# DiWu9/Union-Thesis-SLAM

Hardware: AMD Instinct MI355X
Metric: depth frames/sec (640x480 into 512^3 @ 2 cm dense TSDF; hash alongside) (higher is better)
Workload: dtype f64

## Files before the change

### union-thesis-slam_amd/csrc/tsdf_common.hip

```cpp
#include <unistd.h>

#include <algorithm>
#include <atomic>
#include <chrono>
#include <cmath>
#include <condition_variable>
#include <cstring>
#include <mutex>
#include <thread>
#include <vector>

#include "tsdf_host.h"

namespace tsdf {

static thread_local std::string g_err;

int set_error(int code, const char* fmt, ...) {
    char buf[1024];
    va_list ap;
    va_start(ap, fmt);
    vsnprintf(buf, sizeof(buf), fmt, ap);
    va_end(ap);
    g_err = buf;
// ... 355 lines not shown
    CopyJob job_;
    std::atomic<unsigned long long> gen_{0};
    std::atomic<int> left_{0}, bad_{0}, sleepers_{0};
    int spin_us_ = 300;
};
}

extern "C" int tsdf_diag_depth_to_mm(const double* src, long long n, unsigned short* dst) {
    if (!src || !dst || n < 0) return set_error(TSDF_E_ARG, "bad arguments");
    return CopyPool::get().depth_mm(dst, src, (size_t)n) ? 1 : 0;
}

static void par_memcpy(void* dst, const void* src, size_t bytes) {
    if (bytes < (4u << 20)) {
        CopyPool::get().copy(dst, src, bytes);
        return;
    }
    const unsigned hw = std::thread::hardware_concurrency();
    const size_t nt = std::min<size_t>(8, hw ? hw : 1);
    std::vector<std::thread> th;
    const size_t chunk = (bytes + nt - 1) / nt;
    for (size_t i = 0; i < nt; ++i) {
        const size_t o = i * chunk;
        if (o >= bytes) break;
        th.emplace_back([=] { std::memcpy((char*)dst + o, (const char*)src + o, std::min(chunk, bytes - o)); });
    }
    for (auto& t : th) t.join();
}

int Base::prepare_batch(Batch* bt, const void* depth, int dk, const void* color, int ck, int H,
                        int W, const double K[9], const double* Tinv, const double* ow,
                        double ow_default, int flags, int first, int n, int slot) {
    TSDF_TRY(ensure_pyr(H, W));
    const size_t npx = (size_t)H * W;
    const size_t dbytes = npx * (dk == TSDF_DEPTH_U16_MM ? 2 : 8);
    const size_t cbytes = npx * (ck == TSDF_COLOR_RGB8 ? 3 : 4);
    const char* d = (const char*)depth + dbytes * (size_t)first;
    const char* c = (const char*)color + cbytes * (size_t)first;
    if (!(flags & TSDF_DEVICE_PTRS)) {
        if (prestaged >= 0) {
            slot = prestaged;
        } else {
            TSDF_TRY(stage_alloc(dbytes, cbytes));
            TSDF_HIP(hipEventSynchronize(ev_copied[slot]));
            par_memcpy(hst_depth[slot], d, dbytes * n);
            par_memcpy(hst_color[slot], c, cbytes * n);
        }
        const size_t c0 = prestaged >= 0 ? (size_t)std::min(pre_copied, n) : 0;
        TSDF_HIP(hipStreamWaitEvent(cstream, ev_free[slot], 0));
        if (c0 < (size_t)n) {
            TSDF_HIP(hipMemcpyAsync((char*)st_depth[slot] + dbytes * c0, (const char*)hst_depth[slot] + dbytes * c0,
                                    dbytes * (n - c0), hipMemcpyHostToDevice, cstream));
            TSDF_HIP(hipMemcpyAsync((char*)st_color[slot] + cbytes * c0, (const char*)hst_color[slot] + cbytes * c0,
                                    cbytes * (n - c0), hipMemcpyHostToDevice, cstream));
        }
        TSDF_HIP(hipEventRecord(ev_copied[slot], cstream));
        TSDF_HIP(hipStreamWaitEvent(stream, ev_copied[slot], 0));
        d = (const char*)st_depth[slot];
        c = (const char*)st_color[slot];
    }
    const bool mask = (flags & TSDF_DEPTH_INVALID_65535) && dk == TSDF_DEPTH_U16_MM;
    if (mask && (dmask_px < npx || !dmask_set[n_sets - 1])) {
        TSDF_TRY(sync_all());
        for (int k = 0; k < kSets; ++k) {
            if (dmask_set[k]) TSDF_HIP(hipFree(dmask_set[k]));
            dmask_set[k] = nullptr;
        }
        for (int k = 0; k < n_sets; ++k)
            TSDF_HIP(hipMalloc(&dmask_set[k], sizeof(unsigned short) * npx * batch));
        dmask_px = npx;
    }
    use_set(cur_set);
    bt->n = n;
    const bool tex = texel_now && dk == TSDF_DEPTH_U16_MM && ck == TSDF_COLOR_RGB8;
    bt->texel = tex ? 1 : 0;
    for (int i = 0; i < n; ++i) {
        Frame* fr = &bt->f[i];
        const double* T = Tinv + 16 * (size_t)(first + i);
        for (int r = 0; r < 12; ++r) fr->T[r] = T[r];
        fr->fx = (double)(float)K[0];
        fr->fy = (double)(float)K[4];
        fr->cx = (double)(float)K[2];
        fr->cy = (double)(float)K[5];
        const double margin = frame_margin(W, H, fr->cx, fr->cy);
        fr->half_m = 0.5 - margin;
        for (int j = 0; j < 4; ++j) {
            fr->Tf[j] = T[j] * fr->fx;
            fr->Tf[4 + j] = T[4 + j] * fr->fy;
        }
        {
            double wmax[3];
            for (int a = 0; a < 3; ++a) {
                const long long gmax = (a == 0 ? (long long)vol.off[0] + col_gx(vol, vol.nb[0] - 1) + kBrickEdge
                                               : (long long)vol.off[a] + vol.dims[a]);
                wmax[a] = fabs((double)vol.origin[a]) + vol.vs * (double)gmax + 1.0;
            }
            const double zmin = fold_bound(T, fr->fx, fr->fy, wmax, margin);
            long long bits;
            std::memcpy(&bits, &zmin, sizeof bits);
            const long long hi = (std::isfinite(zmin) && zmin < 1e300) ? (bits >> 32) + 1 : 0x7FEFFFFFll;
            fr->zmin_hi = (int)std::min<long long>(hi, 0x7FEFFFFFll);
        }
        fr->ow = ow ? ow[first + i] : ow_default;
        fr->ow32 = (float)fr->ow;
        fr->H = H;
        fr->W = W;
        fr->depth_src = d + dbytes * i;
        fr->depth_mask = mask ? dmask + npx * i : nullptr;
        fr->depth = mask ? (const void*)fr->depth_mask : fr->depth_src;
        fr->color = c + cbytes * i;
        const bool direct = ck == TSDF_COLOR_RGB8 && rgb_direct &&
                            (!(flags & TSDF_DEVICE_PTRS) || (call_color_end && (const char*)fr->color + cbytes < call_color_end));
        if (tex) fr->rgbx = rgbx + 2 * npx * i;
        else fr->rgbx = direct ? nullptr : rgbx + npx * i;
        fr->pyr = pyr + (size_t)lay.total * i;

        frustum_planes(fr, T, W, H);
    }
    for (int L = 0; L <= kPyrLevels; ++L) {
        bt->pg.off[L] = lay.off[L];
        bt->pg.w[L] = lay.w[L];
        bt->pg.h[L] = lay.h[L];
    }
    return TSDF_OK;
}

int Base::stage_alloc(size_t dbytes, size_t cbytes) {
    if (st_depth_bytes >= dbytes * batch && st_color_bytes >= cbytes * batch) return TSDF_OK;
    TSDF_TRY(sync_all());
    for (int k = 0; k < kSlots; ++k) {
        if (st_depth[k]) TSDF_HIP(hipFree(st_depth[k]));
        if (st_color[k]) TSDF_HIP(hipFree(st_color[k]));
        if (hst_depth[k]) TSDF_HIP(hipHostFree(hst_depth[k]));
        if (hst_color[k]) TSDF_HIP(hipHostFree(hst_color[k]));
        st_depth[k] = st_color[k] = hst_depth[k] = hst_color[k] = nullptr;
    }
    st_depth_bytes = st_color_bytes = 0;
    for (int k = 0; k < kSlots; ++k) {
        TSDF_HIP(hipMalloc(&st_depth[k], dbytes * batch));
        TSDF_HIP(hipMalloc(&st_color[k], cbytes * batch + 64));
        TSDF_HIP(hipHostMalloc(&hst_depth[k], dbytes * batch, hipHostMallocDefault));
        TSDF_HIP(hipHostMalloc(&hst_color[k], cbytes * batch, hipHostMallocDefault));
    }
    st_depth_bytes = dbytes * batch;
    st_color_bytes = cbytes * batch;
    return TSDF_OK;
}

bool Base::defer_same(int dk, int ck, int H, int W, const double* K) const {
    return dfr.dk_in == dk && dfr.ck == ck && dfr.H == H && dfr.W == W && std::memcmp(dfr.K, K, sizeof(dfr.K)) == 0;
}

int Base::defer_push(const void* depth, int dk, const void* color, int ck, int H, int W,
                     const double* K, const double* T, double ow) {
    const size_t cbytes = frame_bytes_color(ck, H, W), npx = (size_t)H * W;
    if (dfr.n == 0) {
        TSDF_TRY(stage_alloc(frame_bytes_depth(dk, H, W), cbytes));
        dfr.slot = defer_next;
        dfr.copied = 0;
        defer_next = (defer_next + 1) % kSlots;
        TSDF_HIP(hipEventSynchronize(ev_copied[dfr.slot]));
        dfr.dk_in = dk;
        dfr.dk = dk;
        dfr.ck = ck;
        dfr.H = H;
        dfr.W = W;
        std::memcpy(dfr.K, K, sizeof(dfr.K));
    }
    const int i = dfr.n;
    const bool try_mm = i == 0 ? mm_backoff == 0 : dfr.dk == TSDF_DEPTH_U16_MM;
    if (i == 0 && mm_backoff > 0) --mm_backoff;
    char* const cdst = (char*)hst_color[dfr.slot] + cbytes * i;
    if (dk == TSDF_DEPTH_F64_M && defer_mm && try_mm) {
        if (CopyPool::get().frame(true, (unsigned short*)hst_depth[dfr.slot] + npx * i, depth, npx, cdst, color,
                                  cbytes)) {
            dfr.dk = TSDF_DEPTH_U16_MM;
        } else {
            mm_backoff = kMmBackoff;
            if (i > 0) return kDeferFlush;
            dfr.dk = TSDF_DEPTH_F64_M;
            CopyPool::get().copy(hst_depth[dfr.slot], depth, frame_bytes_depth(dfr.dk, H, W));
        }
    } else {
        const size_t db = frame_bytes_depth(dfr.dk, H, W);
// ... 231 lines not shown
```

### union-thesis-slam_amd/csrc/tsdf_device.h

```cpp
#pragma once
#include <hip/hip_runtime.h>
#include <stdint.h>
#include <type_traits>

namespace tsdf {

constexpr int kBrickEdge = 8;
constexpr int kBrickVox = 512;
constexpr int kWG = 256;
constexpr int kPyrLevels = 6;
constexpr int kStatSpread = 64;
constexpr unsigned long long kEmpty = ~0ull;
constexpr unsigned long long kTomb = ~0ull - 1ull;

enum Stat { ST_VOXELS = 0, ST_VISITED, ST_TOUCHED, ST_ALLOC, ST_PROBE, ST_LOOKUPS, ST_OVERFLOW,
            ST_PROBE_MAX, ST_BAD_ENTRY, ST_UNIQUE, kNStat };

struct Vol {
    int dims[3];
    int off[3];
    int xstride;
    int xodd;
    int sb[3];
    int nb[3];
    int shard, n_shards;
    int canon;
    float origin[3];
    double vs, trunc;
    double rtrunc;
    const double* rcp;
};

__host__ __device__ inline int col_gx(const Vol& v, int c) {
    return (c >> 1) * 2 * v.xstride + (c & 1) * v.xodd;
}

struct Frame {
    double T[12];
    double fx, fy, cx, cy;
    double ow;
    double half_m;
    double Tf[8];
    int zmin_hi;
    float ow32;
    int H, W;
    const void* depth;
    const void* depth_src;
    unsigned short* depth_mask;
    const void* color;
    const unsigned* rgbx;
    const float* pyr;
    float planes[5][4];
    double eye[3];
};

struct PyrGeo {
    int off[kPyrLevels + 1];
    int w[kPyrLevels + 1];
    int h[kPyrLevels + 1];
};

#ifndef TSDF_MAX_BATCH
#define TSDF_MAX_BATCH 32
#endif
constexpr int kMaxBatch = TSDF_MAX_BATCH;
static_assert(kMaxBatch == 8 || kMaxBatch == 16 || kMaxBatch == 32, "frames per batch: 8, 16 or 32");
#ifndef TSDF_FULL_BATCH
#define TSDF_FULL_BATCH TSDF_MAX_BATCH
#endif
constexpr int kFullBatch = TSDF_FULL_BATCH < kMaxBatch ? TSDF_FULL_BATCH : kMaxBatch;
constexpr int kDoneWord = kMaxBatch + 8, kDoneWordC = kMaxBatch + 9, kCursorWord = kMaxBatch + 10;
constexpr int kCountWords = kMaxBatch + 16;
constexpr int kRcpTab = 4096;
constexpr int kRcpBig = 65536;

__device__ inline bool small_int(float w) {
    return w >= 0.0f && w < (float)(kRcpTab - kMaxBatch - 1) && w == truncf(w);
}
__device__ inline bool table_int(float w) {
    return w >= 0.0f && w < (float)(kRcpBig - kMaxBatch - 1) && w == truncf(w);
}
__device__ inline bool canon_color(float c) {
    return c >= 0.0f && c < 16777216.0f && c == truncf(c);
}
struct Batch {
    Frame f[kMaxBatch];
    PyrGeo pg;
    int n;
    int texel;
};

typedef unsigned long long ListEntry;

struct Pool {
    float* tsdf;
    float* weight;
    float* color;
};

struct PoolState {
    long long pool_top;
    long long free_count;
    long long cursor;
    long long n_overflow;
    long long tombs;
    long long n_inserted;
};

constexpr int kReports = 8;
struct PoolReport {
    long long pool_top, free_count, n_overflow;
    long long listed;
    long long tombs;
    long long seq;
};

struct Table {
    unsigned long long* keys;
    int* vals;
    unsigned long long* occ;
    int* free_list;
    ListEntry* overflow;
    PoolState* st;
    PoolReport* rb;
    long long capacity;
    long long shard_cap;
    long long max_blocks;
    const int* owned;
    int n_owned;
    int* ins_list;
    long long ins_cap;
    int overflow_cap;
    int int_bits;
};

template <bool POW2 = false>
__host__ __device__ inline long long ref_hash(long long x, long long y, long long z, long long n,
                                              int int_bits) {
    const unsigned long long P1 = 73856093ull, P2 = 19349669ull, P3 = 83492791ull;
    long long h;
    if (int_bits == 32) {
        const int a = (int)(unsigned)((unsigned long long)x * P1);
        const int b = (int)(unsigned)((unsigned long long)y * P2);
        const int c = (int)(unsigned)((unsigned long long)z * P3);
        h = (long long)(a ^ b ^ c);
    } else {
        h = (long long)(((unsigned long long)x * P1) ^ ((unsigned long long)y * P2) ^
                        ((unsigned long long)z * P3));
    }
    if (POW2 || (n & (n - 1)) == 0) return h & (n - 1);
    long long m = h % n;
    return m < 0 ? m + n : m;
}

template <bool POW2 = false>
__host__ __device__ inline int shard_of(long long home, int n_shards, long long cap) {
    if (POW2 || (cap & (cap - 1)) == 0) return (int)((home * n_shards) >> (63 - __builtin_clzll((unsigned long long)cap)));
    return (int)((home * n_shards) / cap);
}

__host__ __device__ inline unsigned long long pack_key(int bx, int by, int bz) {
    return (unsigned long long)bx | ((unsigned long long)by << 21) | ((unsigned long long)bz << 42);
}

__device__ inline int lane_id() { return threadIdx.x & 63; }

__device__ unsigned long long fcmp64_mask(double a, double b, int pred) __asm("llvm.amdgcn.fcmp.i64.f64");
__device__ unsigned long long fcmp32_mask(float a, float b, int pred) __asm("llvm.amdgcn.fcmp.i64.f32");
__device__ unsigned long long icmp32_mask(unsigned a, unsigned b, int pred) __asm("llvm.amdgcn.icmp.i64.i32");
constexpr int kCmpOGT = 2, kCmpOGE = 3, kCmpOLT = 4, kCmpUNE = 14, kCmpNE = 33, kCmpULT = 36, kCmpSGT = 38;
__device__ inline bool lane_in(unsigned long long m) { return __builtin_amdgcn_inverse_ballot_w64(m); }
__device__ inline void sel_in_place(float& x, float y, unsigned long long m) {
    asm("v_cndmask_b32 %0, %0, %1, %2" : "+v"(x) : "v"(y), "s"(m));
}

template <typename T>
__device__ inline T coh_load(T* p) {
    return __hip_atomic_load(p, __ATOMIC_RELAXED, __HIP_MEMORY_SCOPE_AGENT);
}
template <typename T>
__device__ inline void coh_store(T* p, T v) {
    __hip_atomic_store(p, v, __ATOMIC_RELAXED, __HIP_MEMORY_SCOPE_AGENT);
}

__device__ inline double vox_world(float origin, double vs, int g) {
    return (double)(float)((double)origin + vs * (double)g);
}

struct BrickBox {
    double p0[3];
    float ext[3];
    float ctr[3];
    float rad;
};

__device__ inline BrickBox brick_box(const Vol& v, const double* eye, int bx, int by, int bz, int nx = 1,
                                     int ny = 1, int nz = 1) {
    const int bb[3] = {bx, by, bz}, nn[3] = {nx, ny, nz};
    BrickBox r;
#pragma unroll
    for (int a = 0; a < 3; ++a) {
        const int lo = bb[a] * kBrickEdge;
        const int hi = min(lo + nn[a] * kBrickEdge - 1, v.dims[a] - 1);
        const int glo = (a == 0) ? col_gx(v, bb[0]) : lo;
        const int ghi = (a == 0) ? col_gx(v, hi >> 3) + (hi & 7) : hi;
        r.p0[a] = (double)v.origin[a] + v.vs * (double)(glo + v.off[a]);
        r.ext[a] = (float)(v.vs * (double)(ghi - glo));
        r.ctr[a] = (float)(r.p0[a] + 0.5 * v.vs * (double)(ghi - glo) - eye[a]);
    }
    r.rad = 0.5f * sqrtf(r.ext[0] * r.ext[0] + r.ext[1] * r.ext[1] + r.ext[2] * r.ext[2]) + 1e-4f;
    return r;
}

__device__ inline bool cull_brick(const Vol& v, const Frame& fr, const PyrGeo& pg, const BrickBox& bb) {
#pragma unroll
    for (int i = 0; i < 5; ++i) {
        const float* q = fr.planes[i];
        if (q[0] * bb.ctr[0] + q[1] * bb.ctr[1] + q[2] * bb.ctr[2] + q[3] < -bb.rad) return false;
    }
    const double* T = fr.T;
    float c0[3], d[3][3];
#pragma unroll
    for (int r = 0; r < 3; ++r) {
        c0[r] = (float)(T[4 * r + 0] * bb.p0[0] + T[4 * r + 1] * bb.p0[1] + T[4 * r + 2] * bb.p0[2] + T[4 * r + 3]);
#pragma unroll
        for (int a = 0; a < 3; ++a) d[r][a] = (float)T[4 * r + a] * bb.ext[a];
    }
    const float fx = (float)fr.fx, fy = (float)fr.fy, cx = (float)fr.cx, cy = (float)fr.cy;
    float zmin = 3e38f, zmax = -3e38f, umin = 3e38f, umax = -3e38f, vmin = 3e38f, vmax = -3e38f;
#pragma unroll
    for (int c = 0; c < 8; ++c) {
        float q[3];
#pragma unroll
        for (int r = 0; r < 3; ++r)
            q[r] = c0[r] + ((c & 1) ? d[r][0] : 0.0f) + ((c & 2) ? d[r][1] : 0.0f) + ((c & 4) ? d[r][2] : 0.0f);
        zmin = fminf(zmin, q[2]);
        zmax = fmaxf(zmax, q[2]);
        const float iz = __builtin_amdgcn_rcpf(fmaxf(q[2], 1e-6f));
        const float u = fx * q[0] * iz + cx, w = fy * q[1] * iz + cy;
        umin = fminf(umin, u); umax = fmaxf(umax, u);
        vmin = fminf(vmin, w); vmax = fmaxf(vmax, w);
    }
    if (zmax < -1e-4f) return false;
    int u0 = 0, u1 = fr.W - 1, v0 = 0, v1 = fr.H - 1;
    if (zmin > 0.2f) {
        const float fu0 = floorf(umin) - 1.0f, fu1 = ceilf(umax) + 1.0f;
        const float fv0 = floorf(vmin) - 1.0f, fv1 = ceilf(vmax) + 1.0f;
        if (fu1 < 0.0f || fv1 < 0.0f || fu0 > (float)(fr.W - 1) || fv0 > (float)(fr.H - 1)) return false;
        u0 = (int)fmaxf(fu0, 0.0f); u1 = (int)fminf(fu1, (float)(fr.W - 1));
        v0 = (int)fmaxf(fv0, 0.0f); v1 = (int)fminf(fv1, (float)(fr.H - 1));
    }
    int L = 1;
    while (L < kPyrLevels && (((u1 >> L) - (u0 >> L)) > 3 || ((v1 >> L) - (v0 >> L)) > 3)) ++L;
// ... 44 lines not shown
        unsigned long long tm = __ballot(kk == kTomb);
        if (emp) tm &= (emp & (~emp + 1)) - 1;
        if (tomb < 0 && tm) tomb = __shfl(s, __ffsll((long long)tm) - 1);
        if (emp) {
            if (!insert) return -1;
            const int le = __ffsll((long long)emp) - 1;
            const long long target = tomb >= 0 ? tomb : __shfl(s, le);
            const unsigned long long expect = tomb >= 0 ? kTomb : kEmpty;
            int ok = 0;
            if (lane == 0) {
                if (blk < 0) blk = pool_alloc(t);
                if (blk >= 0) {
                    const unsigned long long old = atomicCAS(&t.keys[target], expect, key);
                    if (old == expect) {
                        coh_store(&t.vals[target], blk);
                        ok = 1;
                    } else if (old == key) {
                        ok = 2;
                    }
                }
            }
            blk = __shfl(blk, 0);
            ok = __shfl(ok, 0);
            if (blk == -2) return -1;
            if (ok == 1) {
                is_new = true;
                slot_out = target;
                probe = scanned + ((target - pos + t.capacity) % t.capacity);
                return blk;
            }
            if (ok == 2) {
                slot_out = target;
                probe = scanned + ((target - pos + t.capacity) % t.capacity);
                return coh_load(&t.vals[target]);
            }
            scanned += (target - pos + t.capacity) % t.capacity + 1;
            pos = target + 1;
            if (pos >= t.capacity) pos -= t.capacity;
            tomb = -1;
            continue;
        }
        pos += 64;
        if (pos >= t.capacity) pos -= t.capacity;
        scanned += 64;
    }
    return -1;
}


__device__ unsigned short buf_ld_u16(__amdgpu_buffer_rsrc_t r, int vindex, int voffset, int soffset,
                                     int aux) __asm("llvm.amdgcn.struct.ptr.buffer.load.i16");
__device__ unsigned buf_ld_u32(__amdgpu_buffer_rsrc_t r, int vindex, int voffset, int soffset,
                               int aux) __asm("llvm.amdgcn.struct.ptr.buffer.load.i32");
__device__ double buf_ld_f64(__amdgpu_buffer_rsrc_t r, int vindex, int voffset, int soffset,
                             int aux) __asm("llvm.amdgcn.struct.ptr.buffer.load.f64");
constexpr int kBufDword3 = 0x00020000;
typedef unsigned u32x2 __attribute__((ext_vector_type(2)));
__device__ u32x2 buf_ld_v2u32(__amdgpu_buffer_rsrc_t r, int vindex, int voffset, int soffset,
                              int aux) __asm("llvm.amdgcn.struct.ptr.buffer.load.v2i32");
struct FrameBufs {
    __amdgpu_buffer_rsrc_t depth, color;
};
template <int DK, int CK>
__device__ inline FrameBufs frame_bufs(const Frame& fr) {
    const int n = fr.W * fr.H;
    FrameBufs b;
    if (DK == 2) {
        static_assert(DK != 2 || CK == 0, "texels: RGB8 colour");
        b.depth = b.color = __builtin_amdgcn_make_buffer_rsrc((void*)fr.rgbx, 8, n, kBufDword3);
        return b;
    }
    b.depth = __builtin_amdgcn_make_buffer_rsrc((void*)fr.depth, DK == 0 ? 2 : 8, n, kBufDword3);
    if (CK == 0 && !fr.rgbx) b.color = __builtin_amdgcn_make_buffer_rsrc((void*)fr.color, 3, n, kBufDword3);
    else b.color = __builtin_amdgcn_make_buffer_rsrc((void*)(CK == 0 ? (const void*)fr.rgbx : fr.color), 4, n, kBufDword3);
    return b;
}
template <int DK>
__device__ inline unsigned depth_raw(const FrameBufs& fb, unsigned p) {
    return DK == 0 ? (unsigned)buf_ld_u16(fb.depth, (int)p, 0, 0, 0) : 0u;
}
template <int DK>
__device__ inline double depth_m(const FrameBufs& fb, unsigned p, unsigned raw) {
    if (DK != 1) {
        const double m = (double)raw;
        return fma(m, 0.001, m * -2.0858186326137145e-20);
    }
    return buf_ld_f64(fb.depth, (int)p, 0, 0, 0);
}

__device__ inline double div_rn(double a, double b, double y) {
    const double q0 = a * y;
    const double r = fma(-q0, b, a);
    return fma(r, y, q0);
}

__device__ inline float div_rn32(float a, float b, float y) {
    const float q0 = a * y;
    const float r = fmaf(-q0, b, a);
    return fmaf(r, y, q0);
}

typedef float f2 __attribute__((ext_vector_type(2)));
__device__ inline f2 pk_fma(f2 a, f2 b, f2 c) { return __builtin_elementwise_fma(a, b, c); }
__device__ inline f2 rint2(f2 a) { return f2{rintf(a.x), rintf(a.y)}; }
__device__ inline f2 div_rn32x2(f2 a, f2 b, f2 y) {
    const f2 q0 = a * y;
    const f2 r = pk_fma(-q0, b, a);
    return pk_fma(r, y, q0);
}

inline double frame_margin(int W, int H, double cx, double cy) {
    const double span = (double)(W > H ? W : H) + fmax(fabs(cx), fabs(cy));
    return fmax(1e-4, 1e-7 * span);
}

inline double fold_bound(const double* T, double fx, double fy, const double wmax[3], double margin) {
    double e = 0.0;
    for (int r = 0; r < 2; ++r) {
        const double* t = T + 4 * r;
        const double s = fabs(t[0]) * wmax[0] + fabs(t[1]) * wmax[1] + fabs(t[2]) * wmax[2] + fabs(t[3]);
        e = fmax(e, 8.0 * 0x1p-53 * (r == 0 ? fx : fy) * s);
    }
    return 4.0 * e / margin;
}

__device__ inline int cvt_i32_sat(double x) {
    int r;
    asm("v_cvt_i32_f64 %0, %1" : "=v"(r) : "v"(x));
    return r;
}

__device__ inline double readlane_f64(double x, int l) {
    const unsigned long long u = __double_as_longlong(x);
    const unsigned lo = __builtin_amdgcn_readlane((unsigned)u, l);
    const unsigned hi = __builtin_amdgcn_readlane((unsigned)(u >> 32), l);
    return __longlong_as_double(((long long)hi << 32) | lo);
}


#ifdef TSDF_DIAG
__device__ unsigned long long g_ddiag[8];
#define TSDF_DDIAG(i) (lane_id() == 0 ? (void)atomicAdd(&g_ddiag[i], 1ull) : (void)0)
#else
#define TSDF_DDIAG(i) ((void)0)
#endif

template <int DK, int CK, int NZ>
__device__ __forceinline__ void project_part(double trunc, const Frame& fr, double px, double py,
                                             const double* pzs, double pz_l, int zoff, unsigned long long colm,
                                             int nz, unsigned (&cpx)[NZ], double (&diff)[NZ],
                                             unsigned long long (&okm)[NZ]) {
    constexpr int kPz = NZ < 8 ? NZ : 1;
    const double a2 = fma(fr.T[9], py, fr.T[8] * px);
    const double b0 = fma(fr.Tf[1], py, fma(fr.Tf[0], px, fr.Tf[3]));
    const double b1 = fma(fr.Tf[5], py, fma(fr.Tf[4], px, fr.Tf[7]));
    double zc[NZ];
    int iu[NZ], iv[NZ];
    unsigned long long in[NZ], slow[NZ], any_slow = 0;
#pragma unroll
    for (int k = 0; k < NZ; ++k) {
        const double pz = NZ < 8 ? pzs[k % kPz] : readlane_f64(pz_l, k + zoff);
        zc[k] = fr.T[11] + fma(fr.T[10], pz, a2);
    }
    double rzs[NZ];
#pragma unroll
    for (int k = 0; k < NZ; ++k) rzs[k] = __builtin_amdgcn_rcp(zc[k]);
#pragma unroll
    for (int k = 0; k < NZ; ++k) {
        const double pz = NZ < 8 ? pzs[k % kPz] : readlane_f64(pz_l, k + zoff);
        const double z = zc[k], rz = rzs[k];
        const double sx = fma(fma(fr.Tf[2], pz, b0), rz, fr.cx), sy = fma(fma(fr.Tf[6], pz, b1), rz, fr.cy);
        const double ux = rint(sx), uy = rint(sy);
        const unsigned long long fine = fcmp64_mask(fabs(sx - ux), fr.half_m, kCmpOLT) &
                                        fcmp64_mask(fabs(sy - uy), fr.half_m, kCmpOLT) &
                                        icmp32_mask((unsigned)(__double_as_longlong(z) >> 32), (unsigned)fr.zmin_hi, kCmpSGT);
        const unsigned long long col = k < nz ? colm : 0ull;
        in[k] = col & fine;
        iu[k] = cvt_i32_sat(ux);
        iv[k] = cvt_i32_sat(uy);
        slow[k] = col & ~fine;
        any_slow |= slow[k];
    }
    TSDF_DDIAG(0);
    if (any_slow) {
        TSDF_DDIAG(3);
        const double a0 = fma(fr.T[1], py, fr.T[0] * px);
        const double a1 = fma(fr.T[5], py, fr.T[4] * px);
#pragma unroll
        for (int k = 0; k < NZ; ++k) {
            slow[k] &= fcmp64_mask(zc[k], 0.0, kCmpOGT);
            in[k] |= slow[k];
            if (!slow[k] || !lane_in(slow[k])) continue;
            TSDF_DDIAG(2);
            const double pz = NZ < 8 ? pzs[k % kPz] : readlane_f64(pz_l, k + zoff);
            const double x = fr.T[3] + fma(fr.T[2], pz, a0);
            const double y = fr.T[7] + fma(fr.T[6], pz, a1);
            iu[k] = cvt_i32_sat(rint((x * fr.fx) / zc[k] + fr.cx));
            iv[k] = cvt_i32_sat(rint((y * fr.fy) / zc[k] + fr.cy));
        }
    }
    unsigned long long cand[NZ];
    unsigned pix[NZ];
    const int W = fr.W, H = fr.H;
#pragma unroll
    for (int k = 0; k < NZ; ++k) {
        cand[k] = in[k] & icmp32_mask((unsigned)iu[k], (unsigned)W, kCmpULT) &
                  icmp32_mask((unsigned)iv[k], (unsigned)H, kCmpULT);
        pix[k] = lane_in(cand[k]) ? __umul24((unsigned)iv[k], (unsigned)W) + (unsigned)iu[k] : 0u;
    }
    const FrameBufs fb = frame_bufs<DK, CK>(fr);
    unsigned draw[NZ];
#pragma unroll
    for (int k = 0; k < NZ; ++k) {
        if (DK == 2) {
            const u32x2 t = buf_ld_v2u32(fb.depth, (int)pix[k], 0, 0, 0);
            draw[k] = t.x;
            cpx[k] = t.y;
        } else {
            draw[k] = depth_raw<DK>(fb, pix[k]);
            cpx[k] = buf_ld_u32(fb.color, (int)pix[k], 0, 0, 0);
        }
    }
    __builtin_amdgcn_sched_barrier(0);
    double dep[NZ];
#pragma unroll
    for (int k = 0; k < NZ; ++k) dep[k] = depth_m<DK>(fb, pix[k], draw[k]);
#pragma unroll
    for (int k = 0; k < NZ; ++k) {
        diff[k] = dep[k] - zc[k];
        const unsigned long long dpos = DK != 1 ? icmp32_mask(draw[k], 0u, kCmpNE) : fcmp64_mask(dep[k], 0.0, kCmpOGT);
        okm[k] = cand[k] & dpos & fcmp64_mask(diff[k], -trunc, kCmpOGE);
    }
}

__device__ inline double dist_of(double trunc, double rtrunc, double diff) {
    return fmin(div_rn(diff, trunc, rtrunc), 1.0);
}

constexpr int kResFree = -1, kResFail = -3;

template <bool HASH, int DK, int CK, bool OW1, int NZ, bool CU = false>
__device__ inline void integrate_brick(const Vol& v, const Batch& bt, const Pool& pool,
                                       const Table& tab, ListEntry entry, int zoff,
                                       unsigned long long* s_stat, const double* s_rcp,
                                       unsigned& nupd, unsigned& nuniq, int* res = nullptr) {
    static_assert(!CU || (CK == 0 && OW1), "u32 colour registers: RGB8 frames, obs_weight 1");
    static_assert(NZ == 8 || NZ == 4, "z-parts of 8 or 4 steps");
    constexpr bool kHalfHash = HASH && NZ == 4;
    const int lane = lane_id();
    const int b = __builtin_amdgcn_readfirstlane((int)(entry & 0xFFFFFFFFull));
    const unsigned fmask = __builtin_amdgcn_readfirstlane((unsigned)(entry >> 32));
    const double trunc = v.trunc, rtrunc = v.rtrunc;
    const double* const rcp_hbm = v.rcp;
    const bool canon = CU || v.canon != 0;
    const int nb12 = v.nb[1] * v.nb[2];
    if (b >= v.nb[0] * nb12) {
        if (lane == 0) atomicAdd(&s_stat[ST_BAD_ENTRY], 1ull);
        return;
    }
    const int bx = b / nb12;
    const int rem = b - bx * nb12;
    const int by = rem / v.nb[2];
    const int bz = rem - by * v.nb[2];
    const int lx = bx * kBrickEdge + (lane >> 3);
    const int ly = by * kBrickEdge + (lane & 7);
    const unsigned long long colm = __ballot(lx < v.dims[0] && ly < v.dims[1]);
    const int nz = min(kBrickEdge, v.dims[2] - bz * kBrickEdge) - zoff;
    const double px = vox_world(v.origin[0], v.vs, v.off[0] + col_gx(v, bx) + (lane >> 3));
    const double py = vox_world(v.origin[1], v.vs, v.off[1] + ly);
    const double pz_l = vox_world(v.origin[2], v.vs, v.off[2] + bz * kBrickEdge + (lane & 7));
    constexpr int kPz = NZ < 8 ? NZ : 1;
    double pzs[kPz];
#pragma unroll
    for (int k = 0; k < kPz; ++k) {
        pzs[k] = readlane_f64(pz_l, k + zoff);
        if (NZ < 8) asm("" : "+v"(pzs[k]));
    }

    typename std::conditional<HASH, int, long long>::type blk = HASH ? -1 : b;
    bool is_new = false;
    bool upd = false;
    if constexpr (kHalfHash) {
        const int cur = __builtin_amdgcn_readfirstlane(res[b]);
        if (cur == kResFail) {
            if (zoff == 0 && lane == 0) {
                const unsigned long long o = atomicAdd((unsigned long long*)&tab.st->n_overflow, 1ull);
                if ((long long)o < tab.overflow_cap) tab.overflow[o] = entry;
                atomicAdd(&s_stat[ST_OVERFLOW], 1ull);
            }
            return;
        }
        if (cur < 0 || cur >= tab.max_blocks) {
            if (lane == 0) atomicAdd(&s_stat[ST_BAD_ENTRY], 1ull);
            return;
        }
        blk = cur;
    }
    float ws[NZ], ts[NZ], cs[NZ];
#pragma unroll
    for (int k = 0; k < NZ; ++k) {
        ws[k] = 0.0f;
        ts[k] = 1.0f;
        cs[k] = 0.0f;
    }
    constexpr int kH = NZ / 4;
    unsigned long long loaded[kH];
#pragma unroll
    for (int h = 0; h < kH; ++h) loaded[h] = 0;
    unsigned long long touched[NZ] = {};
    bool w_small = true;
    bool w_table = true;
    bool c_canon = true;
    bool fast_t = OW1 && s_rcp, table_t = false, fast_c = CK == 0 && fast_t;
// ... 673 lines not shown
#endif
#ifndef TSDF_HASH_WAVES
#define TSDF_HASH_WAVES 4
#endif
template <bool HASH, int DK, int CK, bool OW1, int NZ = 8>
__global__ __launch_bounds__(kWG) __attribute__((amdgpu_waves_per_eu(TSDF_HASH_WAVES))) void k_integrate(Vol v, Batch bt, Pool pool, Table tab,
                                                  unsigned long long* stats, const ListEntry* list,
                                                  unsigned int* count, int n_list) {
    (void)v;
    const Vol& vk = *(const Vol*)opaque((VolP)__builtin_amdgcn_kernarg_segment_ptr());
    __shared__ unsigned long long s_stat[kNStat];
    __shared__ double s_rcp[OW1 ? kRcpTab : 1];
    __shared__ unsigned s_next;
    const int tid = threadIdx.x;
    if (tid < kNStat) s_stat[tid] = 0;
    if (tid == 0) s_next = 0;
    if (OW1)
        for (int i = tid; i < kRcpTab / 2; i += kWG) ((double2*)s_rcp)[i] = ((const double2*)vk.rcp)[i];
    __syncthreads();
    integrate_list<HASH, DK, CK, OW1, NZ>(vk, bt, pool, tab, list, count, n_list,
                                          blockIdx.x * (kWG / 64) + (tid >> 6), gridDim.x * (kWG / 64),
                                          s_stat, OW1 ? s_rcp : nullptr, &s_next, blockIdx.x, gridDim.x);
    __syncthreads();
    flush_stats(s_stat, stats);
}

template <int REDUCE>
__device__ inline void pyr_level(const PyrGeo& pg, float* pyr, int L, const float (*src)[33],
                                 float (*dst)[33], int n, int tx = blockIdx.x, int ty = blockIdx.y) {
    const int t = threadIdx.x;
    if (t < n * n) {
        const int rr = t / n, cc = t - rr * n;
        const float m = fmaxf(fmaxf(src[2 * rr][2 * cc], src[2 * rr][2 * cc + 1]),
                              fmaxf(src[2 * rr + 1][2 * cc], src[2 * rr + 1][2 * cc + 1]));
        dst[rr][cc] = m;
        const int X = tx * n + cc, Y = ty * n + rr;
        if (X < pg.w[L] && Y < pg.h[L]) pyr[pg.off[L] + Y * pg.w[L] + X] = m;
    }
}

template <int DK = 0>
__device__ inline void prep_vec_tile(const Batch& bt, unsigned int* count, int tx, int ty, int tf,
                                     float (*sa)[33], float (*sb)[33]) {
    const Frame& fr = bt.f[tf];
    float* pyr = (float*)fr.pyr;
    const int t = threadIdx.x, r = t >> 4, c = t & 15;
    if (count && t < kCountWords && tx == 0 && ty == 0 && tf == 0) coh_store(count + t, 0u);
    const bool act = t < 512;
    const int x0 = tx * 64 + c * 4, y0 = ty * 64 + r * 2;
    float ma = 0.0f, mb = 0.0f;
    if (act && x0 < fr.W) {
#pragma unroll
        for (int dy = 0; dy < 2; ++dy) {
            const int y = y0 + dy;
            if (y >= fr.H) continue;
            const size_t p = (size_t)y * fr.W + x0;
            uint2 dd = make_uint2(0u, 0u);
            if (DK == 1) {
                const double2 d0 = *(const double2*)((const double*)fr.depth_src + p);
                const double2 d1 = *(const double2*)((const double*)fr.depth_src + p + 2);
                ma = fmaxf(ma, fmaxf((float)d0.x, (float)d0.y));
                mb = fmaxf(mb, fmaxf((float)d1.x, (float)d1.y));
            } else {
                dd = *(const uint2*)((const unsigned short*)fr.depth_src + p);
                if (fr.depth_mask) {
                    unsigned lo0 = dd.x & 0xFFFFu, hi0 = dd.x >> 16, lo1 = dd.y & 0xFFFFu, hi1 = dd.y >> 16;
                    lo0 = lo0 == 65535u ? 0u : lo0;
                    hi0 = hi0 == 65535u ? 0u : hi0;
                    lo1 = lo1 == 65535u ? 0u : lo1;
                    hi1 = hi1 == 65535u ? 0u : hi1;
                    dd = make_uint2(lo0 | (hi0 << 16), lo1 | (hi1 << 16));
                    *(uint2*)(fr.depth_mask + p) = dd;
                }
                ma = fmaxf(ma, fmaxf((float)(dd.x & 0xFFFFu) * 1e-3f, (float)(dd.x >> 16) * 1e-3f));
                mb = fmaxf(mb, fmaxf((float)(dd.y & 0xFFFFu) * 1e-3f, (float)(dd.y >> 16) * 1e-3f));
            }
            if (fr.rgbx) {
                const unsigned* q = (const unsigned*)((const unsigned char*)fr.color + 3 * p);
                const unsigned a = q[0], b = q[1], cc = q[2];
                const uint4 c4 = make_uint4(a & 0xFFFFFFu, (a >> 24) | ((b & 0xFFFFu) << 8),
                                            (b >> 16) | ((cc & 0xFFu) << 16), cc >> 8);
                if (DK == 2) {
                    uint4* t = (uint4*)((uint2*)fr.rgbx + p);
                    t[0] = make_uint4(dd.x & 0xFFFFu, c4.x, dd.x >> 16, c4.y);
                    t[1] = make_uint4(dd.y & 0xFFFFu, c4.z, dd.y >> 16, c4.w);
                } else {
                    *(uint4*)((unsigned*)fr.rgbx + p) = c4;
                }
            }
        }
    }
    const PyrGeo& pg = bt.pg;
    const auto put = [&](int L, int X, int Y, float m) {
        if (X < pg.w[L] && Y < pg.h[L]) pyr[pg.off[L] + Y * pg.w[L] + X] = m;
    };
    if (act) {
        const int X = x0 >> 1, Y = y0 >> 1;
        put(1, X, Y, ma);
        put(1, X + 1, Y, mb);
    }
    float m2 = fmaxf(ma, mb);
    m2 = fmaxf(m2, __shfl_down(m2, 16));
    if (act && (r & 1) == 0) put(2, tx * 16 + c, ty * 16 + (r >> 1), m2);
    float m3 = fmaxf(m2, __shfl_down(m2, 1));
    m3 = fmaxf(m3, __shfl_down(m3, 32));
    if (act && (r & 3) == 0 && (c & 1) == 0) {
        put(3, tx * 8 + (c >> 1), ty * 8 + (r >> 2), m3);
        sa[r >> 2][c >> 1] = m3;
    }
    __syncthreads();
    if (t < 64) {
        const int lx = t & 7, ly = t >> 3;
        float m = sa[ly][lx];
        m = fmaxf(m, __shfl_down(m, 1));
        m = fmaxf(m, __shfl_down(m, 8));
        if ((lx & 1) == 0 && (ly & 1) == 0) put(4, tx * 4 + (lx >> 1), ty * 4 + (ly >> 1), m);
        m = fmaxf(m, __shfl_down(m, 2));
        m = fmaxf(m, __shfl_down(m, 16));
        if ((lx & 3) == 0 && (ly & 3) == 0) put(5, tx * 2 + (lx >> 2), ty * 2 + (ly >> 2), m);
        m = fmaxf(m, __shfl_down(m, 4));
        m = fmaxf(m, __shfl_down(m, 32));
        if (t == 0) put(6, tx, ty, m);
    }
    (void)sb;
}

template <int DK = 0>
__global__ __launch_bounds__(512) void k_prep_vec(Batch bt, unsigned int* count) {
    __shared__ float sa[32][33];
    __shared__ float sb[32][33];
    prep_vec_tile<DK>(bt, count, blockIdx.x, blockIdx.y, blockIdx.z, sa, sb);
}

template <int DK, int CK>
__global__ __launch_bounds__(1024) void k_prep(Batch bt, unsigned int* count) {
    __shared__ float sa[32][33];
    __shared__ float sb[32][33];
    const Frame& fr = bt.f[blockIdx.z];
    float* pyr = (float*)fr.pyr;
    unsigned* rgbx = (unsigned*)fr.rgbx;
    const int t = threadIdx.x, r = t >> 5, c = t & 31;
    if (count && t < kCountWords && blockIdx.x == 0 && blockIdx.y == 0 && blockIdx.z == 0) coh_store(count + t, 0u);
    const int x0 = blockIdx.x * 64 + c * 2, y0 = blockIdx.y * 64 + r * 2;
    float m1 = 0.0f;
#pragma unroll
    for (int dy = 0; dy < 2; ++dy)
#pragma unroll
        for (int dx = 0; dx < 2; ++dx) {
            const int x = x0 + dx, y = y0 + dy;
            if (x < fr.W && y < fr.H) {
                const int p = y * fr.W + x;
                float d;
                if (DK == 0) {
                    unsigned v = ((const unsigned short*)fr.depth_src)[p];
                    if (fr.depth_mask) {
                        v = (v == 65535u) ? 0u : v;
                        fr.depth_mask[p] = (unsigned short)v;
                    }
                    d = (float)v * 1e-3f;
                } else {
                    d = (float)((const double*)fr.depth_src)[p];
                }
                if (CK == 0 && rgbx) {
                    const unsigned char* q = (const unsigned char*)fr.color + 3 * (size_t)p;
                    const unsigned c = (unsigned)q[0] | ((unsigned)q[1] << 8) | ((unsigned)q[2] << 16);
                    rgbx[p] = c;
                }
                m1 = fmaxf(m1, (float)d);
// ... 220 lines not shown
```

### union-thesis-slam_amd/csrc/tsdf_host.h

```cpp
#pragma once
#include <hip/hip_runtime.h>

#include <cstdarg>
#include <cstdlib>
#include <cstdio>
#include <string>
#include <utility>
#include <vector>

#include "tsdf_device.h"
#include "tsdf_hip.h"

#ifndef TSDF_CULL_WAVES_DEFAULT
#define TSDF_CULL_WAVES_DEFAULT 2
#endif

namespace tsdf {

int set_error(int code, const char* fmt, ...);

#define TSDF_HIP(expr)                                                                        \
    do {                                                                                      \
        hipError_t e_ = (expr);                                                               \
        if (e_ != hipSuccess)                                                                 \
            return ::tsdf::set_error(e_ == hipErrorOutOfMemory ? TSDF_E_OOM : TSDF_E_HIP,     \
                                     "%s failed: %s (%s:%d)", #expr, hipGetErrorString(e_),   \
                                     __FILE__, __LINE__);                                     \
    } while (0)

#define TSDF_TRY(expr)            \
    do {                          \
        int r_ = (expr);          \
        if (r_ != TSDF_OK) return r_; \
    } while (0)

inline size_t frame_bytes_depth(int dk, int H, int W) { return (size_t)H * W * (dk == TSDF_DEPTH_U16_MM ? 2 : 8); }
inline size_t frame_bytes_color(int ck, int H, int W) { return (size_t)H * W * (ck == TSDF_COLOR_RGB8 ? 3 : 4); }

struct PyrLayout {
    int off[kPyrLevels + 1];
    int w[kPyrLevels + 1];
    int h[kPyrLevels + 1];
    int total;
};
PyrLayout pyr_layout(int H, int W);

struct Profiler {
    bool on = false;
    std::vector<std::pair<hipEvent_t, hipEvent_t>> pending;
    std::vector<hipEvent_t> spare;
    double ms = 0.0;
    long long launches = 0;
    int begin(hipStream_t s, hipEvent_t* e0);
    int end(hipStream_t s, hipEvent_t e0);
    int collect();
    void release();
};

constexpr int kSets = 3;
constexpr int kSlots = 4;

struct IcpCtx;
void icp_ctx_free(IcpCtx* c);

struct Base {
    int device = 0;
    hipStream_t stream = nullptr;
    Vol vol{};
    Pool pool{};
    long long n_bricks = 0;
    int batch = kMaxBatch;
    int set_batch(int want);
    int defer_frames = 8;
    int dma_grain = 2;
    bool rgb_direct = true;
    int texel_mode = -1;
    bool texel_now = false;
    static constexpr long long kTexelMinBricksDense = 3ll << 14, kTexelMinBricksHash = 3ll << 15;
    bool texel_for(int dk, long long owned_bricks, long long min_bricks) const {
        if (dk != TSDF_DEPTH_U16_MM) return false;
        return texel_mode >= 0 ? texel_mode != 0 : owned_bricks >= min_bricks;
    }
    bool defer_mm = true;
    int mm_backoff = 0;
    static constexpr int kMmBackoff = 4;
    const char* call_color_end = nullptr;
    float* pyr = nullptr;
    unsigned* rgbx = nullptr;
    int pyr_H = 0, pyr_W = 0;
    ListEntry* list = nullptr;
    unsigned int* count = nullptr;
    float* pyr_set[kSets] = {};
    unsigned* rgbx_set[kSets] = {};
    ListEntry* list_set[kSets] = {};
    unsigned int* count_set[kSets] = {};
    unsigned short* dmask_set[kSets] = {};
    int n_sets = 1;
    int n_cu = 256;
    PyrLayout lay{};
    unsigned long long* stats = nullptr;
    double* rcp = nullptr;
    long long frames = 0;
    Profiler prof;
    hipStream_t cstream = nullptr;
    hipEvent_t ev_copied[kSlots] = {};
    hipEvent_t ev_free[kSlots] = {};
    void* st_depth[kSlots] = {};
    void* st_color[kSlots] = {};
    size_t st_depth_bytes = 0, st_color_bytes = 0;
    unsigned short* dmask = nullptr;
    size_t dmask_px = 0;
    void* hst_depth[kSlots] = {};
    void* hst_color[kSlots] = {};

    struct Deferred {
        int n = 0, H = 0, W = 0, dk = 0, ck = 0, slot = -1;
        int dk_in = 0;
        int copied = 0;
        double K[9];
        double T[16 * kMaxBatch];
        double ow[kMaxBatch];
    } dfr;
    int defer_next = 0;
    int prestaged = -1;
    int pre_copied = 0;
    bool defer_same(int dk, int ck, int H, int W, const double* K) const;
    int defer_push(const void* depth, int dk, const void* color, int ck, int H, int W,
                   const double* K, const double* T, double ow);
    static constexpr int kDeferFlush = 1;
    int stage_alloc(size_t dbytes, size_t cbytes);
    bool stage_fits(int dk, int ck, int H, int W) const {
        return st_depth_bytes >= frame_bytes_depth(dk, H, W) * batch &&
               st_color_bytes >= frame_bytes_color(ck, H, W) * batch;
    }

    int init(int dev, const int64_t dims[3], const int64_t off[3], const float origin[3],
             double vs, double trunc);
    int use_sets(int n);
    int cur_set = 0;
    void use_set(int s) {
        cur_set = s;
        pyr = pyr_set[s];
        rgbx = rgbx_set[s];
        list = list_set[s];
        count = count_set[s];
        dmask = dmask_set[s];
    }
    int sync_all();
    int ensure_pyr(int H, int W);
    int prepare_batch(Batch* bt, const void* depth, int dk, const void* color, int ck, int H,
                      int W, const double K[9], const double* Tinv, const double* ow,
                      double ow_default, int flags, int first, int n, int slot);
    int begin_call(const void* depth, size_t dbytes, const void* color, size_t cbytes, int flags);
    int end_batch(int flags, int slot);
    int end_call(int flags);
    int launch_prep(const Batch& bt, int dk, int ck, int W, int H, hipStream_t st);
    unsigned grid_for(const void* kernel, int wg = kWG);
    unsigned cull_grid() const {
        long long n = 1;
        for (int a = 0; a < 3; ++a) n *= (vol.nb[a] + (1 << vol.sb[a]) - 1) >> vol.sb[a];
        return (unsigned)n;
    }
    int cull_per_wg() const { return cull_grid() >= 1024 ? 3 : 1; }
// ... 79 lines not shown
```

Before: 26280.

## Project voxels to pixels via biased fixed-point doubles and packed u16 bounds checks

Folds the principal point plus a large bias constant into the projection so the low mantissa bits of each projected coordinate directly hold a 16.16 fixed-point pixel value. The rounding-margin test, the image-bounds test and the pixel-index multiply then reduce to packed u16 min/compare and a dot2 instruction, replacing the rint, fabs and compare steps and the separate bounds pass. Texel mode stores invalid depth as a sentinel so the zero-depth check can be dropped for that path. The cost is a more intricate host-side precomputation with extra validity conditions, and a trunc limit that can disable texel mode.

```diff
diff --git a/union-thesis-slam_amd/csrc/tsdf_common.hip b/union-thesis-slam_amd/csrc/tsdf_common.hip
--- a/union-thesis-slam_amd/csrc/tsdf_common.hip
+++ b/union-thesis-slam_amd/csrc/tsdf_common.hip
@@ -461,8 +461,6 @@
         fr->fy = (double)(float)K[4];
         fr->cx = (double)(float)K[2];
         fr->cy = (double)(float)K[5];
-        const double margin = frame_margin(W, H, fr->cx, fr->cy);
-        fr->half_m = 0.5 - margin;
         for (int j = 0; j < 4; ++j) {
             fr->Tf[j] = T[j] * fr->fx;
             fr->Tf[4 + j] = T[4 + j] * fr->fy;
@@ -474,11 +472,13 @@
                                                : (long long)vol.off[a] + vol.dims[a]);
                 wmax[a] = fabs((double)vol.origin[a]) + vol.vs * (double)gmax + 1.0;
             }
-            const double zmin = fold_bound(T, fr->fx, fr->fy, wmax, margin);
-            long long bits;
-            std::memcpy(&bits, &zmin, sizeof bits);
-            const long long hi = (std::isfinite(zmin) && zmin < 1e300) ? (bits >> 32) + 1 : 0x7FEFFFFFll;
-            fr->zmin_hi = (int)std::min<long long>(hi, 0x7FEFFFFFll);
+            const PixelFixed pf = pixel_fixed(T, fr->fx, fr->fy, fr->cx, fr->cy, W, H, wmax);
+            fr->Cx = pf.Cx;
+            fr->Cy = pf.Cy;
+            fr->mm = pf.mm;
+            fr->whm1 = pf.whm1;
+            fr->wmul = pf.wmul;
+            fr->zmin_hi = pf.zmin_hi;
         }
         fr->ow = ow ? ow[first + i] : ow_default;
         fr->ow32 = (float)fr->ow;
diff --git a/union-thesis-slam_amd/csrc/tsdf_device.h b/union-thesis-slam_amd/csrc/tsdf_device.h
--- a/union-thesis-slam_amd/csrc/tsdf_device.h
+++ b/union-thesis-slam_amd/csrc/tsdf_device.h
@@ -2,6 +2,8 @@
 #include <hip/hip_runtime.h>
 #include <stdint.h>
 #include <type_traits>
+
+#include "tsdf_pixel.h"
 
 namespace tsdf {
 
@@ -39,8 +41,9 @@
     double T[12];
     double fx, fy, cx, cy;
     double ow;
-    double half_m;
     double Tf[8];
+    double Cx, Cy;
+    unsigned mm, whm1, wmul;
     int zmin_hi;
     float ow32;
     int H, W;
@@ -168,7 +171,7 @@
 __device__ unsigned long long fcmp64_mask(double a, double b, int pred) __asm("llvm.amdgcn.fcmp.i64.f64");
 __device__ unsigned long long fcmp32_mask(float a, float b, int pred) __asm("llvm.amdgcn.fcmp.i64.f32");
 __device__ unsigned long long icmp32_mask(unsigned a, unsigned b, int pred) __asm("llvm.amdgcn.icmp.i64.i32");
-constexpr int kCmpOGT = 2, kCmpOGE = 3, kCmpOLT = 4, kCmpUNE = 14, kCmpNE = 33, kCmpULT = 36, kCmpSGT = 38;
+constexpr int kCmpOGT = 2, kCmpOGE = 3, kCmpOLT = 4, kCmpUNE = 14, kCmpEQ = 32, kCmpNE = 33, kCmpULT = 36, kCmpSGT = 38;
 __device__ inline bool lane_in(unsigned long long m) { return __builtin_amdgcn_inverse_ballot_w64(m); }
 __device__ inline void sel_in_place(float& x, float y, unsigned long long m) {
     asm("v_cndmask_b32 %0, %0, %1, %2" : "+v"(x) : "v"(y), "s"(m));
@@ -379,7 +382,7 @@
 template <int DK>
 __device__ inline double depth_m(const FrameBufs& fb, unsigned p, unsigned raw) {
     if (DK != 1) {
-        const double m = (double)raw;
+        const double m = DK == 2 ? (double)(int)raw : (double)raw;
         return fma(m, 0.001, m * -2.0858186326137145e-20);
     }
     return buf_ld_f64(fb.depth, (int)p, 0, 0, 0);
@@ -406,25 +409,19 @@
     return pk_fma(r, y, q0);
 }
 
-inline double frame_margin(int W, int H, double cx, double cy) {
-    const double span = (double)(W > H ? W : H) + fmax(fabs(cx), fabs(cy));
-    return fmax(1e-4, 1e-7 * span);
-}
-
-inline double fold_bound(const double* T, double fx, double fy, const double wmax[3], double margin) {
-    double e = 0.0;
-    for (int r = 0; r < 2; ++r) {
-        const double* t = T + 4 * r;
-        const double s = fabs(t[0]) * wmax[0] + fabs(t[1]) * wmax[1] + fabs(t[2]) * wmax[2] + fabs(t[3]);
-        e = fmax(e, 8.0 * 0x1p-53 * (r == 0 ? fx : fy) * s);
-    }
-    return 4.0 * e / margin;
-}
 
 __device__ inline int cvt_i32_sat(double x) {
     int r;
     asm("v_cvt_i32_f64 %0, %1" : "=v"(r) : "v"(x));
     return r;
+}
+
+typedef unsigned short u16x2 __attribute__((ext_vector_type(2)));
+__device__ inline unsigned pk_min_u16(unsigned a, unsigned b) {
+    return __builtin_bit_cast(unsigned, __builtin_elementwise_min(__builtin_bit_cast(u16x2, a), __builtin_bit_cast(u16x2, b)));
+}
+__device__ inline unsigned dot2_u16(unsigned a, unsigned b) {
+    return __builtin_amdgcn_udot2(__builtin_bit_cast(u16x2, a), __builtin_bit_cast(u16x2, b), 0u, false);
 }
 
 __device__ inline double readlane_f64(double x, int l) {
@@ -452,8 +449,8 @@
     const double b0 = fma(fr.Tf[1], py, fma(fr.Tf[0], px, fr.Tf[3]));
     const double b1 = fma(fr.Tf[5], py, fma(fr.Tf[4], px, fr.Tf[7]));
     double zc[NZ];
-    int iu[NZ], iv[NZ];
-    unsigned long long in[NZ], slow[NZ], any_slow = 0;
+    unsigned long long cand[NZ], slow[NZ], any_slow = 0;
+    unsigned pix[NZ];
 #pragma unroll
     for (int k = 0; k < NZ; ++k) {
         const double pz = NZ < 8 ? pzs[k % kPz] : readlane_f64(pz_l, k + zoff);
@@ -466,15 +463,15 @@
     for (int k = 0; k < NZ; ++k) {
         const double pz = NZ < 8 ? pzs[k % kPz] : readlane_f64(pz_l, k + zoff);
         const double z = zc[k], rz = rzs[k];
-        const double sx = fma(fma(fr.Tf[2], pz, b0), rz, fr.cx), sy = fma(fma(fr.Tf[6], pz, b1), rz, fr.cy);
-        const double ux = rint(sx), uy = rint(sy);
-        const unsigned long long fine = fcmp64_mask(fabs(sx - ux), fr.half_m, kCmpOLT) &
-                                        fcmp64_mask(fabs(sy - uy), fr.half_m, kCmpOLT) &
+        const double tx = fma(fma(fr.Tf[2], pz, b0), rz, fr.Cx), ty = fma(fma(fr.Tf[6], pz, b1), rz, fr.Cy);
+        const unsigned lx = (unsigned)__double_as_longlong(tx), ly = (unsigned)__double_as_longlong(ty);
+        const unsigned P = __builtin_amdgcn_perm(ly, lx, 0x05040100u);
+        const unsigned Q = __builtin_amdgcn_perm(ly, lx, 0x07060302u);
+        const unsigned long long fine = icmp32_mask(pk_min_u16(P, fr.mm), fr.mm, kCmpEQ) &
                                         icmp32_mask((unsigned)(__double_as_longlong(z) >> 32), (unsigned)fr.zmin_hi, kCmpSGT);
         const unsigned long long col = k < nz ? colm : 0ull;
-        in[k] = col & fine;
-        iu[k] = cvt_i32_sat(ux);
-        iv[k] = cvt_i32_sat(uy);
+        cand[k] = col & fine & icmp32_mask(pk_min_u16(Q, fr.whm1), Q, kCmpEQ);
+        pix[k] = lane_in(cand[k]) ? dot2_u16(Q, fr.wmul) : 0u;
         slow[k] = col & ~fine;
         any_slow |= slow[k];
     }
@@ -483,27 +480,24 @@
         TSDF_DDIAG(3);
         const double a0 = fma(fr.T[1], py, fr.T[0] * px);
         const double a1 = fma(fr.T[5], py, fr.T[4] * px);
+        const int W = fr.W, H = fr.H;
 #pragma unroll
         for (int k = 0; k < NZ; ++k) {
             slow[k] &= fcmp64_mask(zc[k], 0.0, kCmpOGT);
-            in[k] |= slow[k];
-            if (!slow[k] || !lane_in(slow[k])) continue;
-            TSDF_DDIAG(2);
-            const double pz = NZ < 8 ? pzs[k % kPz] : readlane_f64(pz_l, k + zoff);
-            const double x = fr.T[3] + fma(fr.T[2], pz, a0);
-            const double y = fr.T[7] + fma(fr.T[6], pz, a1);
-            iu[k] = cvt_i32_sat(rint((x * fr.fx) / zc[k] + fr.cx));
-            iv[k] = cvt_i32_sat(rint((y * fr.fy) / zc[k] + fr.cy));
-        }
-    }
-    unsigned long long cand[NZ];
-    unsigned pix[NZ];
-    const int W = fr.W, H = fr.H;
-#pragma unroll
-    for (int k = 0; k < NZ; ++k) {
-        cand[k] = in[k] & icmp32_mask((unsigned)iu[k], (unsigned)W, kCmpULT) &
-                  icmp32_mask((unsigned)iv[k], (unsigned)H, kCmpULT);
-        pix[k] = lane_in(cand[k]) ? __umul24((unsigned)iv[k], (unsigned)W) + (unsigned)iu[k] : 0u;
+            if (!slow[k]) continue;
+            if (lane_in(slow[k])) {
+                TSDF_DDIAG(2);
+                const double pz = NZ < 8 ? pzs[k % kPz] : readlane_f64(pz_l, k + zoff);
+                const double x = fr.T[3] + fma(fr.T[2], pz, a0);
+                const double y = fr.T[7] + fma(fr.T[6], pz, a1);
+                const int iu = cvt_i32_sat(rint((x * fr.fx) / zc[k] + fr.cx));
+                const int iv = cvt_i32_sat(rint((y * fr.fy) / zc[k] + fr.cy));
+                const bool inb = (unsigned)iu < (unsigned)W && (unsigned)iv < (unsigned)H;
+                pix[k] = inb ? __umul24((unsigned)iv, (unsigned)W) + (unsigned)iu : ~0u;
+            }
+            cand[k] |= slow[k] & icmp32_mask(pix[k], ~0u, kCmpNE);
+            pix[k] = lane_in(cand[k]) ? pix[k] : 0u;
+        }
     }
     const FrameBufs fb = frame_bufs<DK, CK>(fr);
     unsigned draw[NZ];
@@ -525,7 +519,7 @@
 #pragma unroll
     for (int k = 0; k < NZ; ++k) {
         diff[k] = dep[k] - zc[k];
-        const unsigned long long dpos = DK != 1 ? icmp32_mask(draw[k], 0u, kCmpNE) : fcmp64_mask(dep[k], 0.0, kCmpOGT);
+        const unsigned long long dpos = DK == 2 ? ~0ull : DK == 0 ? icmp32_mask(draw[k], 0u, kCmpNE) : fcmp64_mask(dep[k], 0.0, kCmpOGT);
         okm[k] = cand[k] & dpos & fcmp64_mask(diff[k], -trunc, kCmpOGE);
     }
 }
@@ -1365,8 +1359,9 @@
                                             (b >> 16) | ((cc & 0xFFu) << 16), cc >> 8);
                 if (DK == 2) {
                     uint4* t = (uint4*)((uint2*)fr.rgbx + p);
-                    t[0] = make_uint4(dd.x & 0xFFFFu, c4.x, dd.x >> 16, c4.y);
-                    t[1] = make_uint4(dd.y & 0xFFFFu, c4.z, dd.y >> 16, c4.w);
+                    const auto dw = [](unsigned d) { return d ? d : TSDF_TEXEL_INVALID; };
+                    t[0] = make_uint4(dw(dd.x & 0xFFFFu), c4.x, dw(dd.x >> 16), c4.y);
+                    t[1] = make_uint4(dw(dd.y & 0xFFFFu), c4.z, dw(dd.y >> 16), c4.w);
                 } else {
                     *(uint4*)((unsigned*)fr.rgbx + p) = c4;
                 }
diff --git a/union-thesis-slam_amd/csrc/tsdf_host.h b/union-thesis-slam_amd/csrc/tsdf_host.h
--- a/union-thesis-slam_amd/csrc/tsdf_host.h
+++ b/union-thesis-slam_amd/csrc/tsdf_host.h
@@ -79,6 +79,7 @@
     static constexpr long long kTexelMinBricksDense = 3ll << 14, kTexelMinBricksHash = 3ll << 15;
     bool texel_for(int dk, long long owned_bricks, long long min_bricks) const {
         if (dk != TSDF_DEPTH_U16_MM) return false;
+        if (!(vol.trunc < TSDF_TEXEL_MAX_TRUNC)) return false;
         return texel_mode >= 0 ? texel_mode != 0 : owned_bricks >= min_bricks;
     }
     bool defer_mm = true;
diff --git a/union-thesis-slam_amd/csrc/tsdf_pixel.h b/union-thesis-slam_amd/csrc/tsdf_pixel.h
--- /dev/null
+++ b/union-thesis-slam_amd/csrc/tsdf_pixel.h
@@ -0,0 +1,87 @@
+#ifndef TSDF_PIXEL_H
+#define TSDF_PIXEL_H
+#include <limits.h>
+#include <math.h>
+#include <string.h>
+
+static inline double frame_margin(int W, int H, double cx, double cy) {
+    const double span = (double)(W > H ? W : H) + fmax(fabs(cx), fabs(cy));
+    return fmax(1e-4, 1e-7 * span);
+}
+
+static inline void fold_rows(const double* T, double fx, double fy, const double wmax[3], double out[2]) {
+    for (int r = 0; r < 2; ++r) {
+        const double* t = T + 4 * r;
+        out[r] = (r == 0 ? fx : fy) *
+                 (fabs(t[0]) * wmax[0] + fabs(t[1]) * wmax[1] + fabs(t[2]) * wmax[2] + fabs(t[3]));
+    }
+}
+
+static inline double fold_bound(const double* T, double fx, double fy, const double wmax[3], double margin) {
+    double b[2];
+    fold_rows(T, fx, fy, wmax, b);
+    return 4.0 * (8.0 * 0x1p-53 * fmax(b[0], b[1])) / margin;
+}
+
+#define TSDF_PIXEL_BIAS 0x1.8p36
+
+typedef struct {
+    double Cx, Cy;
+    unsigned mm;
+    unsigned whm1;
+    unsigned wmul;
+    int zmin_hi;
+    int mx, my;
+    double zmin;
+} PixelFixed;
+
+static inline int pixel_axis(double c, double margin, double* C) {
+    const double C0 = (c + 0.5) + TSDF_PIXEL_BIAS;
+    const double err = fabs(((C0 - TSDF_PIXEL_BIAS) - 0.5) - c);
+    double m = ceil((margin + 0x1p-17 + err) * 65536.0);
+    while (m * 0x1p-16 - 0x1p-17 - err < margin) m += 1.0;
+    *C = C0 + m * 0x1p-16;
+    return m < 32768.0 ? (int)m : -1;
+}
+
+static inline PixelFixed pixel_fixed(const double* T, double fx, double fy, double cx, double cy, int W,
+                                     int H, const double wmax[3]) {
+    PixelFixed p;
+    memset(&p, 0, sizeof p);
+    p.zmin_hi = INT_MAX;
+    p.zmin = INFINITY;
+    int finite = isfinite(fx) && isfinite(fy) && isfinite(cx) && isfinite(cy);
+    for (int r = 0; r < 12; ++r) finite = finite && isfinite(T[r]);
+    for (int j = 0; j < 4; ++j) finite = finite && isfinite(T[j] * fx) && isfinite(T[4 + j] * fy);
+    if (!finite || W < 1 || H < 1 || W > 16384 || H > 16384) return p;
+    const double margin = frame_margin(W, H, cx, cy);
+    double b[2];
+    fold_rows(T, fx, fy, wmax, b);
+    const double denx = 65536.0 - (double)W - fabs(cx) - 2.0, deny = 65536.0 - (double)H - fabs(cy) - 2.0;
+    if (!(denx >= 1.0) || !(deny >= 1.0)) return p;
+    const double zmin = fmax(fold_bound(T, fx, fy, wmax, margin), fmax(b[0] / denx, b[1] / deny));
+    double Cx, Cy;
+    const int mx = pixel_axis(cx, margin, &Cx), my = pixel_axis(cy, margin, &Cy);
+    if (mx < 0 || my < 0 || !isfinite(zmin) || !(zmin < 1e300)) return p;
+    long long bits;
+    memcpy(&bits, &zmin, sizeof bits);
+    p.zmin_hi = (int)(bits >> 32) + 1;
+    p.zmin = zmin;
+    p.Cx = Cx;
+    p.Cy = Cy;
+    p.mx = mx;
+    p.my = my;
+    p.mm = ((unsigned)(2 * my) << 16) | (unsigned)(2 * mx);
+    p.whm1 = ((unsigned)(H - 1) << 16) | (unsigned)(W - 1);
+    p.wmul = ((unsigned)W << 16) | 1u;
+    return p;
+}
+
+#define TSDF_TEXEL_INVALID 0x80000000u
+#define TSDF_TEXEL_MAX_TRUNC 1.0e6
+static inline double texel_depth_m(int raw) {
+    const double m = (double)raw;
+    return fma(m, 0.001, m * -2.0858186326137145e-20);
+}
+
+#endif
```

After: 26900 (median of 6 runs). 2.4% higher.
